# zhaihongjia/SplatLoc

Measured on AMD Instinct MI355X. Metric: fwd+bwd frames/s @1080p, 500k Gaussians, 32 feat-ch; HBM GB/s vs roofline, higher is better.
Workload: dtype f32

## Files before the change

### include/splatraster.h

```cpp
#ifndef SPLATRASTER_H
#define SPLATRASTER_H

#include <stddef.h>
#include <stdint.h>

#ifdef __cplusplus
extern "C" {
#endif

#define SPLATRASTER_ABI_VERSION 20

#define SPLATRASTER_TILE 16

#define SPLATRASTER_OK 0
#define SPLATRASTER_ERR_BAD_ARG 1
#define SPLATRASTER_ERR_HIP 2
#define SPLATRASTER_ERR_UNSUPPORTED 3
#define SPLATRASTER_ERR_OVERFLOW 4
#define SPLATRASTER_WARN_LOOKBACK_STALL 5

typedef struct splatraster_settings {
    int32_t image_height;
    int32_t image_width;
    float tanfovx;
// ... 160 lines not shown
    float* dL_drotation;
    float* dL_dopacity;
    float* dL_df_dc;
    float* dL_dextra;
    const float* reg_row_grad;
    const float* reg_out;
    float reg_weight;
} splatraster_raw_params;
int splatraster_backward_window_raw(const splatraster_settings* s, int32_t n_views, const splatraster_window_view* views,
                                    int32_t P, const int64_t* num_rendered, const float* bg, const float* means3D,
                                    const float* colors_precomp, const float* scales, const float* rotations, void* geometry,
                                    const void* binning, const void* image, const splatraster_raw_params* raw,
                                    float* dL_dmeans3D , void* stream);

typedef struct splatraster_bounded_status {
    uint32_t total;
    uint32_t overflow;
    uint32_t first_tag;
    uint32_t first_total;
    uint32_t last_tag;
    uint32_t reserved[11];
} splatraster_bounded_status;
int splatraster_bounded_status_create(void** handle);
int splatraster_bounded_status_destroy(void* handle);
int splatraster_bounded_status_read(const void* handle, splatraster_bounded_status* out);
int splatraster_bounded_status_clear(void* handle, void* stream);
int splatraster_forward_window_bounded_supported(int32_t P, int32_t n_views, int32_t width, int32_t height);
int splatraster_forward_window_bounded(const splatraster_settings* s, int32_t n_views, const splatraster_window_view* views,
                                       int32_t P, const float* means3D, const float* opacities, const float* scales,
                                       const float* rotations, const float* cov3D_precomp, const float* bg,
                                       const float* colors_precomp, void* geometry, void* binning, void* image,
                                       int64_t capacity, uint32_t tag, void* status, void* stream);
int splatraster_forward_window_bounded_raw(const splatraster_settings* s, int32_t n_views, const splatraster_window_view* views,
                                           int32_t P, const float* means3D, const splatraster_raw_forward* raw, const float* bg,
                                           void* geometry, void* binning, void* image, int64_t capacity, uint32_t tag,
                                           void* status, void* stream);


int splatraster_mark_visible(int32_t P, const float* means3D, const float* viewmatrix,
                             const float* projmatrix, uint8_t* present, void* stream);

typedef struct splatraster_geometry_layout {
    size_t rec0;
    size_t rec1;
    size_t tiles_touched;
    size_t depth_order;
    size_t offsets;
    size_t rgb;
    size_t clamped;
    size_t total;
} splatraster_geometry_layout;
typedef struct splatraster_binning_layout {
    size_t point_list;
    size_t tile_list;
    size_t ranges;
    size_t total;
} splatraster_binning_layout;
typedef struct splatraster_image_layout {
    size_t final_T;
    size_t n_contrib;
    size_t total;
} splatraster_image_layout;
int splatraster_get_geometry_layout(int32_t P, splatraster_geometry_layout* out);
int splatraster_get_binning_layout(int32_t P, int64_t R, int32_t width, int32_t height, int32_t channels,
                                   splatraster_binning_layout* out);
int splatraster_get_image_layout(int32_t width, int32_t height, splatraster_image_layout* out);
int splatraster_get_window_geometry_layout(int32_t P, int32_t n_views, splatraster_geometry_layout* out);
int splatraster_get_window_binning_layout(int32_t P, int32_t n_views, int64_t R_total, int32_t width, int32_t height,
                                          int32_t channels, splatraster_binning_layout* out);
int splatraster_get_window_image_layout(int32_t width, int32_t height, int32_t n_views, splatraster_image_layout* out);

size_t splatraster_sort_tmp_bytes(int64_t n);
int splatraster_sort_pairs_u32(int64_t n, uint32_t* keys, uint32_t* vals, int32_t key_bits,
                               void* tmp, void* stream);


int splatraster_debug_sort_path(int64_t n, int32_t key_bits, int32_t keys16);
int splatraster_debug_scan_path(int64_t n);
size_t splatraster_debug_scan_tmp_bytes(int64_t n);
int splatraster_debug_scan_u32(int64_t n, const uint32_t* in, const uint32_t* perm, uint32_t* out, uint64_t* total,
                               int32_t exclusive, uint32_t* span_owner, uint32_t span, uint32_t span_cap, void* tmp,
                               void* stream);
int splatraster_debug_sort_pairs_k16(int64_t n, uint32_t* keys, uint32_t* vals, int32_t key_bits, void* tmp, void* stream);


int splatraster_activate_forward(int32_t P, int32_t sh_coeffs, int32_t active_sh_degree,
                                 int32_t scaling_cols, int32_t extras,
                                 const float* xyz, const float* f_dc, const float* f_rest,
                                 const float* scaling, const float* rotation, const float* opacity,
                                 const float* extra, const float* campos,
                                 float* scales , float* rotations ,
                                 float* opacities , float* colors ,
                                 void* stream);
int splatraster_activate_backward(int32_t P, int32_t sh_coeffs, int32_t active_sh_degree,
                                  int32_t scaling_cols, int32_t extras,
                                  const float* xyz, const float* f_dc, const float* f_rest,
                                  const float* scaling, const float* rotation, const float* opacity,
                                  const float* campos,
                                  const float* dL_dscales, const float* dL_drotations,
                                  const float* dL_dopacities, const float* dL_dcolors,
                                  float* dL_dxyz, float* dL_df_dc, float* dL_df_rest, float* dL_dscaling,
                                  float* dL_drotation, float* dL_dopacity, float* dL_dextra, void* stream);

int splatraster_densification_stats(int32_t P, const float* viewspace_grad , const int32_t* radii,
                                    float* xyz_gradient_accum , float* denom ,
                                    float* max_radii2D , void* stream);
int splatraster_densification_stats_window(int32_t P, int32_t n_views, const float* const* viewspace_grads,
                                           const int32_t* const* radii, float* xyz_gradient_accum, float* denom,
                                           float* max_radii2D, void* stream);


typedef struct splatraster_model {
    int32_t P;
    int32_t f_rest_width;
    int32_t marker_width;
    int32_t kp_width;
    int32_t scaling_width;
    float* xyz;
    float* f_dc;
    float* f_rest;
    float* opacity;
    float* marker;
    float* kp_score;
    float* scaling;
    float* rotation;
} splatraster_model;

size_t splatraster_densify_workspace_bytes(int32_t P);
int splatraster_densify_plan(const splatraster_model* model, const float* xyz_gradient_accum ,
                             const float* denom , float max_grad, float min_opacity, float extent,
                             float percent_dense, int32_t use_size_prune, int32_t primitive_reg, void* workspace,
                             int32_t* new_P, void* stream);
int splatraster_densify_plan_thresholds(const splatraster_model* model, const float* xyz_gradient_accum ,
                                        const float* denom , float max_grad, float min_opacity,
                                        float size_split, float size_prune, int32_t use_size_prune,
                                        int32_t primitive_reg, void* workspace, int32_t* new_P, void* stream);
int splatraster_densify_apply(const splatraster_model* model, const splatraster_model* exp_avg ,
                              const splatraster_model* exp_avg_sq , const float* unit_noise ,
                              uint64_t seed, uint64_t draw_id, void* workspace , int32_t new_P,
                              splatraster_model* out_model, splatraster_model* out_exp_avg,
                              splatraster_model* out_exp_avg_sq, int32_t* source_row ,
                              int32_t* source_kind ,
                              void* stream);

int splatraster_model_append(const splatraster_model* model, const splatraster_model* exp_avg ,
                             const splatraster_model* exp_avg_sq , const splatraster_model* extra,
                             splatraster_model* out_model, splatraster_model* out_exp_avg,
                             splatraster_model* out_exp_avg_sq, void* stream);

typedef struct splatraster_adam_group {
    float* param;
    const float* grad;
    float* exp_avg;
    float* exp_avg_sq;
    const float* row_gate;
    int64_t numel;
    int32_t row_width;
    float lr;
    double step;
} splatraster_adam_group;
int splatraster_adam_step(int32_t n_groups, const splatraster_adam_group* groups, double beta1, double beta2, double eps,
                          float row_gate_threshold, void* stream);
int splatraster_adam_step_radii(int32_t n_groups, const splatraster_adam_group* groups, double beta1, double beta2, double eps,
                                float row_gate_threshold, int32_t P, const int32_t* radii, float* max_radii2D, void* stream);

int splatraster_adam_step_gated(int32_t n_groups, const splatraster_adam_group* groups, double beta1, double beta2, double eps,
// ... 285 lines not shown
```

### splatloc_amd/_native.py

```python
from __future__ import annotations

import ctypes as C
import os

from . import build as _build

_LIB = None
ABI_VERSION = 20
ERR_UNSUPPORTED = 3

OK = 0
WARN_LOOKBACK_STALL = 5
_ERR_NAMES = {1: "bad argument", 2: "HIP runtime error", 3: "unsupported configuration",
              4: "tile instance count overflow", 5: "look-back stall (results late, never wrong)"}


class Settings(C.Structure):
    _fields_ = [
        ("image_height", C.c_int32),
        ("image_width", C.c_int32),
        ("tanfovx", C.c_float),
        ("tanfovy", C.c_float),
        ("scale_modifier", C.c_float),
        ("sh_degree", C.c_int32),
# ... 74 lines not shown


class GridLayout(C.Structure):
    _fields_ = [("n_dims", C.c_int32), ("n_levels", C.c_int32), ("n_features", C.c_int32), ("grid_type", C.c_int32),
                ("offset", C.c_uint32 * GRID_MAX_LEVELS), ("size", C.c_uint32 * GRID_MAX_LEVELS),
                ("resolution", C.c_uint32 * GRID_MAX_LEVELS), ("scale", C.c_float * GRID_MAX_LEVELS), ("n_params", C.c_int64)]


DECODER_MAX_LAYERS = 8


class DecoderLayout(C.Structure):
    _fields_ = [("grid", GridLayout), ("bound", (C.c_double * 2) * 3), ("n_layers", C.c_int32),
                ("dims", C.c_int32 * (DECODER_MAX_LAYERS + 1))]


FUSION_MAX_FRAMES = 8
FUSION_MAX_FEAT_DIM = 256


class FusionVolume(C.Structure):
    _fields_ = [("dim", C.c_int32 * 3), ("feat_dim", C.c_int32), ("axis", C.c_void_p * 3), ("tsdf", C.c_void_p),
                ("weight", C.c_void_p), ("color", C.c_void_p), ("feat", C.c_void_p)]


_vp, _i32, _i64, _sz = C.c_void_p, C.c_int32, C.c_int64, C.c_size_t
SYMBOLS = {
    "splatraster_geometry_bytes": (_sz, [_i32]),
    "splatraster_binning_bytes": (_sz, [_i32, _i64, _i32, _i32, _i32]),
    "splatraster_image_bytes": (_sz, [_i32, _i32]),
    "splatraster_forward_geometry": (C.c_int, [C.POINTER(Settings), _i32] + [_vp] * 9 + [_vp, _vp, C.POINTER(_i64), _vp]),
    "splatraster_forward_render": (C.c_int, [C.POINTER(Settings), _i32, _i64] + [_vp] * 9),
    "splatraster_backward": (C.c_int, [C.POINTER(Settings), _i32, _i64] + [_vp] * 33),
    "splatraster_window_geometry_bytes": (_sz, [_i32, _i32]),
    "splatraster_window_binning_bytes": (_sz, [_i32, _i32, _i64, _i32, _i32, _i32]),
    "splatraster_window_image_bytes": (_sz, [_i32, _i32, _i32]),
    "splatraster_forward_window_geometry": (C.c_int, [C.POINTER(Settings), _i32, C.POINTER(WindowView), _i32] + [_vp] * 6
                                            + [C.POINTER(_i64), _vp]),
    "splatraster_forward_window_render": (C.c_int, [C.POINTER(Settings), _i32, C.POINTER(WindowView), _i32, C.POINTER(_i64)]
                                          + [_vp] * 6),
    "splatraster_backward_window": (C.c_int, [C.POINTER(Settings), _i32, C.POINTER(WindowView), _i32, C.POINTER(_i64)]
                                    + [_vp] * 16),
    "splatraster_window_camera_workspace_bytes": (_sz, [_i32]),
    "splatraster_backward_window_cameras": (C.c_int, [C.POINTER(Settings), _i32, C.POINTER(WindowView), _i32, C.POINTER(_i64)]
                                            + [_vp] * 14),
    "splatraster_backward_window_joint": (C.c_int, [C.POINTER(Settings), _i32, C.POINTER(WindowView), _i32, C.POINTER(_i64)]
                                          + [_vp] * 20),
    "splatraster_forward_window_geometry_raw": (C.c_int, [C.POINTER(Settings), _i32, C.POINTER(WindowView), _i32, _vp, C.POINTER(RawForward),
                                                          _vp, C.POINTER(_i64), _vp]),
    "splatraster_backward_window_raw": (C.c_int, [C.POINTER(Settings), _i32, C.POINTER(WindowView), _i32, C.POINTER(_i64)]
                                        + [_vp] * 8 + [C.POINTER(RawParams)] + [_vp] * 2),
    "splatraster_bounded_status_create": (C.c_int, [C.POINTER(_vp)]),
    "splatraster_bounded_status_destroy": (C.c_int, [_vp]),
    "splatraster_bounded_status_read": (C.c_int, [_vp, C.POINTER(BoundedStatus)]),
    "splatraster_bounded_status_clear": (C.c_int, [_vp, _vp]),
    "splatraster_forward_window_bounded_supported": (C.c_int, [_i32, _i32, _i32, _i32]),
    "splatraster_forward_window_bounded": (C.c_int, [C.POINTER(Settings), _i32, C.POINTER(WindowView), _i32] + [_vp] * 10
                                           + [_i64, C.c_uint32, _vp, _vp]),
    "splatraster_forward_window_bounded_raw": (C.c_int, [C.POINTER(Settings), _i32, C.POINTER(WindowView), _i32, _vp,
                                                         C.POINTER(RawForward)] + [_vp] * 4 + [_i64, C.c_uint32, _vp, _vp]),
    "splatraster_get_window_geometry_layout": (C.c_int, [_i32, _i32, C.POINTER(GeometryLayout)]),
    "splatraster_get_window_binning_layout": (C.c_int, [_i32, _i32, _i64, _i32, _i32, _i32, C.POINTER(BinningLayout)]),
    "splatraster_get_window_image_layout": (C.c_int, [_i32, _i32, _i32, C.POINTER(ImageLayout)]),
    "splatraster_debug_set_small_panel_max_waves": (C.c_int, [C.c_int]),
    "splatraster_debug_set_split_max_waves": (C.c_int, [C.c_int]),
    "splatraster_debug_set_fwd_team": (C.c_int, [C.c_int]),
    "splatraster_debug_set_front_end": (C.c_int, [C.c_int]),
    "splatraster_debug_set_tile_sort_cap": (C.c_int, [C.c_int]),
    "splatraster_debug_set_sort_fork": (C.c_int, [C.c_int]),
    "splatraster_debug_set_payload_stream_min": (C.c_int, [C.c_int64]),
    "splatraster_debug_set_payload_compact": (C.c_int, [C.c_int]),
    "splatraster_debug_set_dead_marks": (C.c_int, [C.c_int]),
    "splatraster_mark_visible": (C.c_int, [_i32, _vp, _vp, _vp, _vp, _vp]),
    "splatraster_get_geometry_layout": (C.c_int, [_i32, C.POINTER(GeometryLayout)]),
    "splatraster_get_binning_layout": (C.c_int, [_i32, _i64, _i32, _i32, _i32, C.POINTER(BinningLayout)]),
    "splatraster_get_image_layout": (C.c_int, [_i32, _i32, C.POINTER(ImageLayout)]),
    "splatraster_sort_tmp_bytes": (_sz, [_i64]),
    "splatraster_sort_pairs_u32": (C.c_int, [_i64, _vp, _vp, _i32, _vp, _vp]),
    "splatraster_debug_sort_path": (C.c_int, [_i64, _i32, _i32]),
    "splatraster_debug_scan_path": (C.c_int, [_i64]),
    "splatraster_debug_scan_tmp_bytes": (_sz, [_i64]),
    "splatraster_debug_scan_u32": (C.c_int, [_i64, _vp, _vp, _vp, _vp, _i32, _vp, C.c_uint32, C.c_uint32, _vp, _vp]),
    "splatraster_debug_sort_pairs_k16": (C.c_int, [_i64, _vp, _vp, _i32, _vp, _vp]),
    "splatraster_timing_enable": (C.c_int, [C.c_int]),
    "splatraster_timing_select": (C.c_int, [C.c_uint32]),
    "splatraster_timing_collect": (C.c_int, [_vp, _vp]),
    "splatknn_workspace_bytes": (_sz, [_i32]),
    "splatknn_dist2": (C.c_int, [_i32, _vp, _vp, _vp, _vp]),
    "splatknn_debug_set_grid_min": (C.c_int, [_i32]),
    "splatraster_grid_encoding_layout": (C.c_int, [_i32] * 5 + [C.c_double, _i32, C.POINTER(GridLayout)]),
    "splatraster_grid_encoding_forward": (C.c_int, [C.POINTER(GridLayout), _i64, _vp, _vp, _vp, _vp]),
    "splatraster_grid_encoding_backward": (C.c_int, [C.POINTER(GridLayout), _i64] + [_vp] * 6),
    "splatraster_decoder_workspace_bytes": (C.c_int, [C.POINTER(DecoderLayout), _i64, C.POINTER(_sz), C.POINTER(_sz)]),
    "splatraster_decoder_forward": (C.c_int, [C.POINTER(DecoderLayout), _i64, _vp, _i32, _vp, C.POINTER(_vp), _vp, _vp, _vp]),
    "splatraster_decoder_backward": (C.c_int, [C.POINTER(DecoderLayout), _i64, _vp, C.POINTER(_vp)] + [_vp] * 9),
    "splatraster_decoder_adam": (C.c_int, [C.POINTER(DecoderLayout), C.POINTER(_vp)] + [_vp] * 7 + [_i64] + [C.c_double] * 7 + [_vp]),
    "splatraster_landmark_scores": (C.c_int, [_i64, _i32] + [_vp] * 4 + [_i32, _i32] + [_vp] * 7),
    "splatraster_landmark_workspace_bytes": (_sz, [_i64, _i32]),
    "splatraster_landmark_select": (C.c_int, [_i64, _vp, _vp, _i32, C.c_double, _vp, _vp, _vp, _vp]),
    "splatraster_fusion_bytes": (C.c_int, [_i32] * 4 + [C.POINTER(_sz), C.POINTER(_sz)]),
    "splatraster_fusion_integrate": (C.c_int, [C.POINTER(FusionVolume), _i32, _i32, _i32] + [_vp] * 5 + [C.c_float, C.c_float, _vp]),
    "splatraster_fusion_surface_count": (C.c_int, [C.POINTER(FusionVolume), _i32, C.c_float, _vp, C.POINTER(_i64), _vp]),
    "splatraster_fusion_surface_extract": (C.c_int, [C.POINTER(FusionVolume), _vp, C.c_double, _vp, _i64] + [_vp] * 6),
    "splatraster_fusion_mesh_bytes": (C.c_int, [_i32] * 3 + [C.POINTER(_sz)]),
    "splatraster_fusion_mesh_count": (C.c_int, [C.POINTER(FusionVolume), _vp, _vp, C.POINTER(_i64), _vp]),
    "splatraster_fusion_mesh_extract": (C.c_int, [C.POINTER(FusionVolume), _vp, _vp, _i64, _i64, _vp, _vp, _vp]),
    "splatraster_debug_mc_table": (C.c_int, [_vp]),
    "splatraster_image_gradient": (C.c_int, [_i32] * 4 + [_vp, C.c_float, _vp, _vp, _vp, _vp]),
    "splatraster_grad_mask_workspace_bytes": (C.c_int, [_i32] * 5 + [C.POINTER(_sz)]),
    "splatraster_grad_mask": (C.c_int, [_i32] * 3 + [_vp, C.c_float, C.c_float, _i32, _i32, _vp, _vp, _vp, _vp, _sz, _vp]),
    "splatraster_debug_image_ops_path": (C.c_int, [_i32, _i32]),
    "splatraster_masked_median_workspace_bytes": (C.c_int, [_i32, _i64, C.POINTER(_sz)]),
    "splatraster_masked_median": (C.c_int, [_i32, _i64, _vp, _i32, _vp, C.c_float, _vp, _vp, _vp, _vp, _vp, _vp, _sz, _vp]),
    "splatraster_sp_nms_tile": (C.c_int, [C.POINTER(_i32), C.POINTER(_i32)]),
    "splatraster_sp_workspace_bytes": (C.c_int, [_i32] * 4 + [C.POINTER(_sz)]),
    "splatraster_sp_scores": (C.c_int, [_i32] * 3 + [_vp, _vp, _vp]),
    "splatraster_sp_nms": (C.c_int, [_i32] * 3 + [_vp, _i32, _vp, _vp]),
    "splatraster_sp_select": (C.c_int, [_i32] * 3 + [_vp, C.c_float, _i32, _i32] + [_vp] * 5 + [_sz, _vp]),
    "splatraster_sp_sample": (C.c_int, [_i32] * 3 + [_vp, _i32] + [_vp] * 4 + [_sz, _vp]),
    "splatraster_sp_dense_descriptors": (C.c_int, [_i32] * 3 + [_vp, _i32, _i32, _vp, _vp, _sz, _vp]),
    "splatraster_lsap_workspace_bytes": (_sz, [_i32, _vp]),
    "splatraster_lsap": (C.c_int, [_i32, _vp, _vp, _i32] + [_vp] * 6),
    "splatraster_debug_set_lsap_lds": (C.c_int, [C.c_int]),
    "splatraster_match_cost": (C.c_int, [_i32, _i32, _i32, _vp, _vp, C.c_float, _vp, _vp, _vp]),
    "splatraster_match_sims": (C.c_int, [_i32, _i32, _i32, _vp, _vp, _vp, C.c_float, _i64, _vp, _vp, _vp, _vp]),
    "splatraster_frustum_workspace_bytes": (_sz, [_i64, _i32, _i32]),
    "splatraster_frustum_candidates": (C.c_int, [_i64, _vp, _vp, C.c_float, _vp, _vp, _i32, _i32] + [_vp] * 10),
    "splatraster_pnp_workspace_bytes": (_sz, [_i32, _vp, _vp]),
    "splatraster_pnp": (C.c_int, [_i32] + [_vp] * 12),
    "splatraster_pnp_hypotheses": (C.c_int, [_i32, _vp, _vp, _i64, _i32] + [_vp] * 7),
    "splatraster_pnp_score": (C.c_int, [_i32, _vp, _vp, _i32] + [_vp] * 7),
    "splatraster_retrieval_workspace_bytes": (_sz, [_i64, _i64, _i32, _i32]),
    "splatraster_retrieval_topk": (C.c_int, [_i64, _i64, _i32, _i32] + [_vp] * 7),
    "splatraster_pose_errors": (C.c_int, [_i64] + [_vp] * 8),
    "splatraster_pose_invert": (C.c_int, [_i64] + [_vp] * 5),
    "splatraster_activate_forward": (C.c_int, [_i32] * 5 + [_vp] * 13),
    "splatraster_activate_backward": (C.c_int, [_i32] * 5 + [_vp] * 19),
    "splatraster_densification_stats": (C.c_int, [_i32] + [_vp] * 6),
    "splatraster_densification_stats_window": (C.c_int, [_i32, _i32] + [_vp] * 6),
    "splatraster_densify_workspace_bytes": (_sz, [_i32]),
    "splatraster_densify_plan": (C.c_int, [C.POINTER(Model), _vp, _vp, C.c_float, C.c_float, C.c_float, C.c_float, _i32,
                                           _i32, _vp, C.POINTER(_i32), _vp]),
    "splatraster_densify_plan_thresholds": (C.c_int, [C.POINTER(Model), _vp, _vp, C.c_float, C.c_float, C.c_float,
                                                      C.c_float, _i32, _i32, _vp, C.POINTER(_i32), _vp]),
    "splatraster_densify_apply": (C.c_int, [C.POINTER(Model), C.POINTER(Model), C.POINTER(Model), _vp, C.c_uint64,
                                            C.c_uint64, _vp, _i32, C.POINTER(Model), C.POINTER(Model), C.POINTER(Model),
                                            _vp, _vp, _vp]),
    "splatraster_model_append": (C.c_int, [C.POINTER(Model)] * 7 + [_vp]),
    "splatraster_adam_step": (C.c_int, [_i32, C.POINTER(AdamGroup), C.c_double, C.c_double, C.c_double, C.c_float, _vp]),
    "splatraster_adam_step_radii": (C.c_int, [_i32, C.POINTER(AdamGroup), C.c_double, C.c_double, C.c_double, C.c_float, _i32, _vp, _vp, _vp]),
    "splatraster_adam_step_gated": (C.c_int, [_i32, C.POINTER(AdamGroup), C.c_double, C.c_double, C.c_double, C.c_float, _vp, _vp]),
    "splatraster_adam_step_radii_gated": (C.c_int, [_i32, C.POINTER(AdamGroup), C.c_double, C.c_double, C.c_double, C.c_float, _i32, _vp,
                                                    _vp, _vp, _vp]),
    "splatraster_isotropic_loss_workspace_bytes": (_sz, [_i32]),
    "splatraster_isotropic_loss": (C.c_int, [_i32, _i32, _vp, _vp, _vp, _vp, _vp, _vp]),
    "splatraster_mapping_loss_workspace_bytes": (_sz, [_i32]),
    "splatraster_mapping_loss": (C.c_int, [_i32] + [_vp] * 6 + [C.c_float] + [_vp] * 7),
    "splatraster_mapping_loss_window": (C.c_int, [_i32, _i32, _vp, C.c_float, _vp, _vp, _vp]),
    "splatraster_refinement_loss_workspace_bytes": (_sz, [_i32, _i32, _i32]),
    "splatraster_refinement_loss": (C.c_int, [_i32, _i32, _i32, C.c_float] + [_vp] * 6),
    "splatraster_eval_metrics_workspace_bytes": (_sz, [_i32, _i32, _i32]),
    "splatraster_eval_metrics": (C.c_int, [_i32, _i32, _i32] + [_vp] * 5),
    "splatraster_l1_rgbd_loss": (C.c_int, [_i64, _vp, _vp, _i64, _vp, _vp, C.c_float, _vp, _vp, _vp, _vp]),
    "splatraster_pose_step": (C.c_int, [_vp] * 5 + [C.c_float] * 5 + [C.c_int] + [_vp] * 5),
    "splatraster_l1_rgbd_loss_window": (C.c_int, [_i32, C.POINTER(L1View), _i64, _i64, C.c_float, _vp, _vp]),
    "splatraster_pose_step_window": (C.c_int, [_i32] + [_vp] * 5 + [C.c_float] * 5 + [C.c_int] + [_vp] * 5),
# ... 120 lines not shown
```

### splatloc_amd/csrc/binning.hip

```cpp
#include "tile_order.h"
#include "composite_common.h"

namespace sr {

__device__ __forceinline__ int f2i_sat_b(float v)
{
    if (!(v > -1.0e9f)) v = -1.0e9f;
    if (!(v < 1.0e9f)) v = 1.0e9f;
    return (int)v;
}

constexpr int EMIT_BLOCK = 256;
constexpr int EMIT_IPT = 4;
static_assert(EMIT_SPAN == EMIT_BLOCK * EMIT_IPT, "common.h: EMIT_SPAN");

template <typename KeyT>
__global__ void __launch_bounds__(EMIT_BLOCK)
emit_kernel(int64_t R, int P , int Pv , int tiles_per_view, int W, int H,
            const uint32_t* __restrict__ offsets,
            const uint32_t* __restrict__ depth_order, const float4* __restrict__ rec,
            KeyT* __restrict__ keys, uint32_t* __restrict__ vals,
            const uint32_t* __restrict__ span_owner ,
            uint32_t* __restrict__ ranges, uint32_t nranges )
{
    for (uint32_t w = blockIdx.x * blockDim.x + threadIdx.x; w < nranges; w += gridDim.x * blockDim.x) ranges[w] = 0u;
    __shared__ uint32_t s_off[EMIT_SPAN + 1];
    __shared__ uint32_t s_gid[EMIT_SPAN], s_org[EMIT_SPAN], s_w[EMIT_SPAN];
    __shared__ int s_min;
    const int t = threadIdx.x;
    const int64_t j0 = (int64_t)blockIdx.x * EMIT_SPAN;
    const uint32_t j0u = (uint32_t)j0;
    int lo = 0, hi = P;
    if (span_owner && blockIdx.x < SPAN_OWNER_CAP) {
        lo = (int)span_owner[blockIdx.x];
        hi = lo + 1;
    }
    while (hi - lo > 1) {
        const int n = hi - lo;
        const int step = (n + EMIT_BLOCK - 1) / EMIT_BLOCK;
        if (t == 0) s_min = EMIT_BLOCK;
        __syncthreads();
        const int last = lo + (t + 1) * step - 1;
        if (last >= hi - 1 || offsets[last] > j0u) atomicMin(&s_min, t);
        __syncthreads();
        const int seg = s_min;
        __syncthreads();
        lo = lo + seg * step;
        hi = min(hi, lo + step);
    }
    const int r_lo = lo;
    for (int q = t; q <= EMIT_SPAN; q += EMIT_BLOCK) {
        const int r = r_lo - 1 + q;
        s_off[q] = r < 0 ? 0u : offsets[min(r, P - 1)];
    }
    __syncthreads();
    const int gx = (W + TILE - 1) / TILE, gy = (H + TILE - 1) / TILE;
    const uint32_t j_last = (uint32_t)(min(R, j0 + (int64_t)EMIT_SPAN) - 1);
    int nr;
    {
        int a = 1, b = EMIT_SPAN + 1;
        while (a < b) {
            const int mid = (a + b) >> 1;
            if (s_off[mid] > j_last) b = mid; else a = mid + 1;
        }
        nr = a;
    }
    for (int q = t; q < nr; q += EMIT_BLOCK) {
        const uint32_t g = depth_order[r_lo + q] & 0xFFFFFFu;
        const float4 p = rec[2 * g];
        const float rf = p.w;
        const int rminx = min(gx, max(0, f2i_sat_b((p.x - rf) / (float)TILE)));
        const int rminy = min(gy, max(0, f2i_sat_b((p.y - rf) / (float)TILE)));
        const int rmaxx = min(gx, max(0, f2i_sat_b((p.x + rf + (float)(TILE - 1)) / (float)TILE)));
        s_gid[q] = g;
        const uint32_t v = (P == Pv) ? 0u : g / (uint32_t)Pv;
        s_org[q] = v * (uint32_t)tiles_per_view + (uint32_t)rminy * (uint32_t)gx + (uint32_t)rminx;
        s_w[q] = (uint32_t)(rmaxx - rminx);
    }
    __syncthreads();
#pragma unroll
    for (int it = 0; it < EMIT_IPT; ++it) {
        const int64_t j = j0 + it * EMIT_BLOCK + t;
        if (j < R) {
            const uint32_t ju = (uint32_t)j;
            int a = 1, b = nr + 1;
            while (a < b) {
                const int mid = (a + b) >> 1;
                if (s_off[mid] > ju) b = mid; else a = mid + 1;
            }
            const uint32_t k = ju - s_off[a - 1];
            const uint32_t w = s_w[a - 1];
            const uint32_t row = k / w;
            keys[j] = (KeyT)(s_org[a - 1] + row * (uint32_t)gx + (k - row * w));
            vals[j] = s_gid[a - 1];
        }
    }
}

int launch_emit(const FramePlan& p, int64_t R, const GeomView& g, uint32_t* keys, uint32_t* vals, uint32_t* ranges,
                uint32_t nranges, hipStream_t stream, bool keys16)
{
    if (R == 0) return SPLATRASTER_OK;
    const int64_t blocks = (R + EMIT_SPAN - 1) / EMIT_SPAN;
    const int n = p.P * p.V;
    const uint32_t* owner = scan_state_bytes(n) ? g.span_owner : nullptr;
    if (keys16)
        hipLaunchKernelGGL(emit_kernel<uint16_t>, dim3((unsigned)blocks), dim3(EMIT_BLOCK), 0, stream, R, n, p.P, p.tiles, p.W, p.H,
                           g.offsets, g.depth_order, g.rec, reinterpret_cast<uint16_t*>(keys), vals, owner, ranges, nranges);
    else
        hipLaunchKernelGGL(emit_kernel<uint32_t>, dim3((unsigned)blocks), dim3(EMIT_BLOCK), 0, stream, R, n, p.P, p.tiles, p.W, p.H,
                           g.offsets, g.depth_order, g.rec, keys, vals, owner, ranges, nranges);
    SR_LAUNCH_CHECK();
    return SPLATRASTER_OK;
}

int launch_ranges_clear(int32_t tiles, uint32_t* ranges, hipStream_t stream)
{
    SR_HIP_CHECK(hipMemsetAsync(ranges, 0, sizeof(uint32_t) * 2 * (size_t)tiles, stream));
    return SPLATRASTER_OK;
}

#ifndef SR_PAYLOAD_NT_MIN
#define SR_PAYLOAD_NT_MIN (8ll << 20)
#endif
static int64_t g_payload_stream_min = SR_PAYLOAD_NT_MIN;
void set_payload_stream_min(int64_t instances) { g_payload_stream_min = instances < 0 ? (int64_t)SR_PAYLOAD_NT_MIN : instances; }

template <bool NT>
__global__ void __launch_bounds__(256)
payload_kernel(int64_t R, int gx, int tiles_per_view, int V, const uint32_t* __restrict__ point_list,
               const uint32_t* __restrict__ tile_list, const float4* __restrict__ rec,
               float4* __restrict__ irec, uint32_t* __restrict__ ipack, uint32_t* __restrict__ ranges)
{
    const int64_t j = (int64_t)blockIdx.x * blockDim.x + threadIdx.x;
    if (j >= R) return;
    const uint32_t g = point_list[j], t = tile_list[j];
    const float4 a0 = rec[2 * (size_t)g], a1 = rec[2 * (size_t)g + 1];
    uint32_t tl = t;
#pragma unroll 1
    for (int v = 1; v < V && tl >= (uint32_t)tiles_per_view; ++v) tl -= (uint32_t)tiles_per_view;
    const uint32_t ty = tl / (uint32_t)gx, tx = tl - ty * (uint32_t)gx;
    const float4 c1 = payload_conic(a1);
    const uint32_t m = g | (quadrant_reach_mask(a0, a1, (float)(tx * TILE), (float)(ty * TILE)) << 24);
    if (NT) {
        typedef float f32x4_t __attribute__((ext_vector_type(4)));
        f32x4_t* out = reinterpret_cast<f32x4_t*>(irec) + 2 * j;
        __builtin_nontemporal_store((f32x4_t){a0.x, a0.y, a0.z, a0.w}, out);
        __builtin_nontemporal_store((f32x4_t){c1.x, c1.y, c1.z, c1.w}, out + 1);
        __builtin_nontemporal_store(m, ipack + j);
    } else {
        irec[2 * j] = a0;
        irec[2 * j + 1] = c1;
        ipack[j] = m;
    }
    if (j == 0 || tile_list[j - 1] != t) ranges[2 * t] = (uint32_t)j;
    if (j == R - 1 || tile_list[j + 1] != t) ranges[2 * t + 1] = (uint32_t)(j + 1);
}

int launch_payload(const FramePlan& p, int64_t R, const GeomView& g, const BinView& b, hipStream_t stream)
{
    if (R == 0) return SPLATRASTER_OK;
    if (R >= g_payload_stream_min)
        hipLaunchKernelGGL(payload_kernel<true>, dim3((unsigned)((R + 255) / 256)), dim3(256), 0, stream, R, p.gx, p.tiles, p.V,
                           b.point_list, b.tile_list, g.rec, b.irec, b.ipack, b.ranges);
    else
        hipLaunchKernelGGL(payload_kernel<false>, dim3((unsigned)((R + 255) / 256)), dim3(256), 0, stream, R, p.gx, p.tiles, p.V,
                           b.point_list, b.tile_list, g.rec, b.irec, b.ipack, b.ranges);
    SR_LAUNCH_CHECK();
    return SPLATRASTER_OK;
}

__global__ void __launch_bounds__(256)
ranges_kernel(int64_t R, const uint32_t* __restrict__ tile_list, uint32_t* __restrict__ ranges)
{
    const int64_t j = (int64_t)blockIdx.x * blockDim.x + threadIdx.x;
    if (j >= R) return;
    const uint32_t t = tile_list[j];
    if (j == 0 || tile_list[j - 1] != t) ranges[2 * t] = (uint32_t)j;
    if (j == R - 1 || tile_list[j + 1] != t) ranges[2 * t + 1] = (uint32_t)(j + 1);
}

template <bool NT>
__global__ void __launch_bounds__(256)
payload_tile_kernel(int gx, int tiles_per_view, const uint32_t* __restrict__ ranges, const uint32_t* __restrict__ point_list,
                    const float4* __restrict__ rec, float4* __restrict__ irec, uint32_t* __restrict__ ipack,
// ... 118 lines not shown
```

### splatloc_amd/csrc/capi.hip

```cpp
#include <assert.h>
#include <string.h>

#include <mutex>
#include <unordered_map>
#include <string>
#include <vector>

#include "common.h"

namespace sr {

static thread_local std::string g_last_error;
static int g_deterministic = 0;
static int g_split_max_waves = SPLIT_MAX_WAVES;
static int g_fwd_team = -1;
static int g_payload_compact = -1;
static int g_dead_marks = 1;
static int g_bin_mode = -1;

void set_hip_error(hipError_t e, const char* what)
{
    g_last_error = std::string(what) + ": " + hipGetErrorString(e);
}

// ... 963 lines not shown
    if (P < 0) return SPLATRASTER_ERR_BAD_ARG;
    if (P == 0) return SPLATRASTER_OK;
    if (!means3D || !viewmatrix || !present) return SPLATRASTER_ERR_BAD_ARG;
    return launch_mark_visible(P, means3D, viewmatrix, present, reinterpret_cast<hipStream_t>(stream));
}

int splatraster_poll_errors(void) { return lookback_error_poll(); }

int splatraster_debug_set_deterministic(int on)
{
    g_deterministic = on ? 1 : 0;
    return SPLATRASTER_OK;
}

int splatraster_debug_set_spin_limit(uint32_t limit)
{
    int st = lookback_error_init();
    if (st) return st;
    return lookback_set_spin_limit(limit);
}

int splatraster_debug_exp2(int64_t n, const float* x, float* y, void* stream)
{
    if (n < 0) return SPLATRASTER_ERR_BAD_ARG;
    if (n == 0) return SPLATRASTER_OK;
    if (!x || !y) return SPLATRASTER_ERR_BAD_ARG;
    return launch_debug_exp2(n, x, y, reinterpret_cast<hipStream_t>(stream));
}

int splatraster_debug_poison_lds(uint32_t pattern, void* stream)
{
    return launch_poison_lds(pattern, reinterpret_cast<hipStream_t>(stream));
}

struct SortInPlace { uint32_t *keys_alt, *vals_alt; void* tmp; size_t bytes; };
static SortInPlace sort_in_place_layout(void* base, int64_t n)
{
    const size_t m = (size_t)(n > 0 ? n : 1);
    SortInPlace L;
    Carver c{base};
    L.keys_alt = c.take<uint32_t>(m);
    L.vals_alt = c.take<uint32_t>(m);
    L.tmp = c.take<char>(sort_tmp_bytes(n));
    L.bytes = c.o;
    return L;
}
size_t splatraster_sort_tmp_bytes(int64_t n) { return sort_in_place_layout(nullptr, n).bytes; }

static int sort_in_place(bool keys16, int64_t n, uint32_t* keys, uint32_t* vals, int32_t key_bits, void* tmp, void* stream_)
{
    if (!keys || !vals || !tmp) return SPLATRASTER_ERR_BAD_ARG;
    {
        int st0 = lookback_error_init();
        if (st0) return st0;
    }
    hipStream_t stream = reinterpret_cast<hipStream_t>(stream_);
    const SortInPlace L = sort_in_place_layout(tmp, n);
    uint32_t *ka = L.keys_alt, *va = L.vals_alt;
    bool in_alt = false;
    int st = keys16 ? sort_pairs_k16(n, keys, vals, ka, va, key_bits, L.tmp, stream, &in_alt)
                    : sort_pairs_u32(n, keys, vals, ka, va, key_bits, L.tmp, stream, &in_alt);
    if (st) return st;
    if (in_alt) {
        SR_HIP_CHECK(hipMemcpyAsync(keys, ka, 4 * (size_t)n, hipMemcpyDeviceToDevice, stream));
        SR_HIP_CHECK(hipMemcpyAsync(vals, va, 4 * (size_t)n, hipMemcpyDeviceToDevice, stream));
    }
    return SPLATRASTER_OK;
}

int splatraster_sort_pairs_u32(int64_t n, uint32_t* keys, uint32_t* vals, int32_t key_bits, void* tmp,
                               void* stream_)
{
    if (n < 0 || key_bits < 0 || key_bits > 32) return SPLATRASTER_ERR_BAD_ARG;
    if (n == 0 || key_bits == 0) return SPLATRASTER_OK;
    return sort_in_place(false, n, keys, vals, key_bits, tmp, stream_);
}

int splatraster_debug_sort_pairs_k16(int64_t n, uint32_t* keys, uint32_t* vals, int32_t key_bits, void* tmp, void* stream_)
{
    if (n < 0 || key_bits < 0 || key_bits > 32 || !sort_keys16(n, key_bits)) return SPLATRASTER_ERR_BAD_ARG;
    return sort_in_place(true, n, keys, vals, key_bits, tmp, stream_);
}

int splatraster_debug_sort_path(int64_t n, int32_t key_bits, int32_t keys16)
{
    if (n < 0 || key_bits < 0 || key_bits > 32 || (keys16 && !sort_keys16(n, key_bits))) return -1;
    return sort_path(n, key_bits, keys16 != 0);
}

int splatraster_debug_scan_path(int64_t n) { return n < 0 ? -1 : scan_path(n); }

size_t splatraster_debug_scan_tmp_bytes(int64_t n) { return scan_tmp_bytes(n > 0 ? n : 0); }

int splatraster_debug_scan_u32(int64_t n, const uint32_t* in, const uint32_t* perm, uint32_t* out, uint64_t* total,
                               int32_t exclusive, uint32_t* span_owner, uint32_t span, uint32_t span_cap, void* tmp, void* stream_)
{
    if (n < 0) return SPLATRASTER_ERR_BAD_ARG;
    if (exclusive && (perm || in != out || span_owner)) return SPLATRASTER_ERR_BAD_ARG;
    if (span_owner && span == 0) return SPLATRASTER_ERR_BAD_ARG;
    if (n > 0 && (!in || !out || !tmp)) return SPLATRASTER_ERR_BAD_ARG;
    if (n > 0 && perm && in == out) return SPLATRASTER_ERR_BAD_ARG;
    if (n == 0 && !total) return SPLATRASTER_OK;
    {
        int st0 = lookback_error_init();
        if (st0) return st0;
    }
    hipStream_t stream = reinterpret_cast<hipStream_t>(stream_);
    uint32_t* total32 = reinterpret_cast<uint32_t*>(total);
    if (exclusive) return exclusive_scan_u32(n, out, total32, tmp, stream, false);
    return inclusive_scan_u32(n, in, perm, out, total32, tmp, stream, false, span_owner, span, span_cap);
}

int splatraster_timing_enable(int on)
{
    std::lock_guard<std::mutex> lk(g_timing_mu);
    g_timing_mask = on ? 0xffffffffu : 0u;
    return SPLATRASTER_OK;
}

int splatraster_timing_select(uint32_t stage_mask)
{
    std::lock_guard<std::mutex> lk(g_timing_mu);
    g_timing_mask = stage_mask;
    return SPLATRASTER_OK;
}

int splatraster_timing_collect(double* ms, int64_t* counts)
{
    if (!ms || !counts) return SPLATRASTER_ERR_BAD_ARG;
    std::lock_guard<std::mutex> lk(g_timing_mu);
    for (const StageRec& r : g_recs) {
        SR_HIP_CHECK(hipEventSynchronize(r.b));
        float t = 0.f;
        SR_HIP_CHECK(hipEventElapsedTime(&t, r.a, r.b));
        if (r.stage >= 0 && r.stage < SPLATRASTER_STAGE_COUNT) { ms[r.stage] += (double)t; counts[r.stage] += 1; }
        g_pool.push_back(r.a);
        g_pool.push_back(r.b);
    }
    g_recs.clear();
    return SPLATRASTER_OK;
}

}
```

### splatloc_amd/csrc/scan.h

```cpp
#pragma once
#include "common.h"

namespace sr {

__device__ __forceinline__ uint64_t lanes_below(int lane) { return (lane == 0) ? 0ull : (~0ull >> (WAVE - lane)); }

template <typename T>
__device__ __forceinline__ T wave_inclusive_scan(T v)
{
    static_assert(sizeof(T) == 4 || sizeof(T) == 8, "uint32_t or uint64_t");
    const int lane = threadIdx.x & (WAVE - 1);
#pragma unroll
    for (int d = 1; d < WAVE; d <<= 1) {
        const T t = __shfl_up(v, d, WAVE);
        if (lane >= d) v += t;
    }
    return v;
}

template <int THREADS, typename T>
__device__ __forceinline__ T block_exclusive_scan(T v, T* s_wsum, T* total = nullptr)
{
    constexpr int NW = THREADS / WAVE;
    const int w = __builtin_amdgcn_readfirstlane(threadIdx.x / WAVE);
    const T incl = wave_inclusive_scan(v);
    if ((threadIdx.x & (WAVE - 1)) == WAVE - 1) s_wsum[w] = incl;
    __syncthreads();
    T before = 0, all = 0;
    constexpr int UNROLL = NW <= 4 ? NW : 2;
#pragma unroll UNROLL
    for (int k = 0; k < NW; ++k) {
        const T c = s_wsum[k];
        before += (k < w) ? c : (T)0;
        all += c;
    }
    if (total) *total = all;
    return before + incl - v;
}

__device__ __forceinline__ uint32_t float_order_key(float v)
{
    const uint32_t u = __float_as_uint(v);
    return (u & 0x80000000u) ? ~u : (u | 0x80000000u);
}
__device__ __forceinline__ float float_from_order_key(uint32_t key)
{
    return __uint_as_float((key & 0x80000000u) ? (key ^ 0x80000000u) : ~key);
}

template <bool DESCENDING>
__device__ __forceinline__ void radix_pick(const uint32_t* hist, bool median, uint32_t k, uint32_t* digit, uint32_t* rank, uint32_t* total)
{
    const int lane = threadIdx.x & (WAVE - 1);
    uint32_t c[4];
#pragma unroll
    for (int j = 0; j < 4; ++j) c[j] = hist[DESCENDING ? 255 - (4 * lane + j) : 4 * lane + j];
    const uint32_t s = (c[0] + c[1]) + (c[2] + c[3]);
    const uint32_t incl = wave_inclusive_scan(s);
    const uint32_t tot = __shfl(incl, WAVE - 1);
    if (median) k = tot ? (tot - 1) / 2 : 0;
    const uint32_t excl = incl - s;
    const bool mine = excl <= k && k < incl;
    uint32_t dg = 0, kr = 0;
    if (mine) {
        uint32_t cum = excl;
#pragma unroll
        for (int j = 0; j < 4; ++j) {
            if (k < cum + c[j]) {
                dg = DESCENDING ? 255 - (4 * lane + j) : 4 * lane + j;
                kr = k - cum;
                break;
            }
            cum += c[j];
        }
    }
    const unsigned long long owners = __ballot(mine);
    const int src = owners ? __ffsll((long long)owners) - 1 : 0;
    *digit = __shfl(dg, src);
    *rank = __shfl(kr, src);
    *total = tot;
}

struct plain_barrier {
    __device__ __forceinline__ void operator()() const { __syncthreads(); }
};
template <int THREADS, bool DESCENDING, typename KeyAt, typename FirstBarrier = plain_barrier>
__device__ __forceinline__ uint32_t radix_select_block(uint32_t n, KeyAt key_at, uint32_t k, uint32_t* s_hist, uint32_t* s_sel,
                                                       uint32_t* rank_left = nullptr, FirstBarrier first_barrier = FirstBarrier())
{
    static_assert(THREADS >= 256, "one thread per bin");
    const uint32_t tid = threadIdx.x;
    uint32_t prefix = 0;
    for (int shift = 24; shift >= 0; shift -= 8) {
        if (tid < 256) s_hist[tid] = 0;
        __syncthreads();
        const uint32_t hi = shift == 24 ? 0u : 0xFFFFFFFFu << (shift + 8);
        for (uint32_t i = tid; i < n; i += THREADS) {
            const uint32_t u = key_at(i);
// ... 24 lines not shown
```

Measured before the change: 798.3.

## Replace per-instance binary search in emit with owner-mark max-scan and reciprocal division

The tile-key emit kernel no longer binary-searches the shared offset array for each output slot. Each range start now writes its owner index into a 16-bit shared array, and a wave-level inclusive max-scan plus a cross-wave carry spreads ownership to every slot. The per-instance integer division that splits an index into row and column is replaced by a float reciprocal estimate with a one-step correction when the tile count is small enough. A debug C entry point is added to test emit on its own. The aim is to cut the log-depth shared-memory searches and the slow integer divides. The costs are extra shared-memory passes and barriers, and a new limit on grid width that returns unsupported.

```diff
diff --git a/include/splatraster.h b/include/splatraster.h
--- a/include/splatraster.h
+++ b/include/splatraster.h
@@ -266,6 +266,8 @@
                                int32_t exclusive, uint32_t* span_owner, uint32_t span, uint32_t span_cap, void* tmp,
                                void* stream);
 int splatraster_debug_sort_pairs_k16(int64_t n, uint32_t* keys, uint32_t* vals, int32_t key_bits, void* tmp, void* stream);
+int splatraster_debug_emit(int64_t R, int32_t n, int32_t Pv, int32_t W, int32_t H, const uint32_t* offsets, const uint32_t* depth_order,
+                           const float* rec, uint32_t* keys, uint32_t* vals, int32_t keys16, const uint32_t* span_owner, void* stream);
 
 
 int splatraster_activate_forward(int32_t P, int32_t sh_coeffs, int32_t active_sh_degree,
diff --git a/splatloc_amd/_native.py b/splatloc_amd/_native.py
--- a/splatloc_amd/_native.py
+++ b/splatloc_amd/_native.py
@@ -180,6 +180,7 @@
     "splatraster_debug_scan_tmp_bytes": (_sz, [_i64]),
     "splatraster_debug_scan_u32": (C.c_int, [_i64, _vp, _vp, _vp, _vp, _i32, _vp, C.c_uint32, C.c_uint32, _vp, _vp]),
     "splatraster_debug_sort_pairs_k16": (C.c_int, [_i64, _vp, _vp, _i32, _vp, _vp]),
+    "splatraster_debug_emit": (C.c_int, [_i64, _i32, _i32, _i32, _i32, _vp, _vp, _vp, _vp, _vp, _i32, _vp, _vp]),
     "splatraster_timing_enable": (C.c_int, [C.c_int]),
     "splatraster_timing_select": (C.c_int, [C.c_uint32]),
     "splatraster_timing_collect": (C.c_int, [_vp, _vp]),
diff --git a/splatloc_amd/csrc/binning.hip b/splatloc_amd/csrc/binning.hip
--- a/splatloc_amd/csrc/binning.hip
+++ b/splatloc_amd/csrc/binning.hip
@@ -13,6 +13,18 @@
 constexpr int EMIT_BLOCK = 256;
 constexpr int EMIT_IPT = 4;
 static_assert(EMIT_SPAN == EMIT_BLOCK * EMIT_IPT, "common.h: EMIT_SPAN");
+static_assert(EMIT_SPAN <= 65536 && EMIT_BLOCK == 4 * WAVE, "emit_kernel: 16-bit row numbers, one 64-slot segment per wave and step");
+
+constexpr uint32_t EMIT_RCP_MAX_TILES = 1u << 22;
+__device__ __forceinline__ uint32_t rect_row(uint32_t k, uint32_t w, uint32_t* col)
+{
+    uint32_t row = (uint32_t)(((float)k + 0.5f) * __builtin_amdgcn_rcpf((float)w));
+    int32_t c = (int32_t)(k - row * w);
+    if (c < 0) { row -= 1u; c += (int32_t)w; }
+    else if (c >= (int32_t)w) { row += 1u; c -= (int32_t)w; }
+    *col = (uint32_t)c;
+    return row;
+}
 
 template <typename KeyT>
 __global__ void __launch_bounds__(EMIT_BLOCK)
@@ -25,7 +37,9 @@
 {
     for (uint32_t w = blockIdx.x * blockDim.x + threadIdx.x; w < nranges; w += gridDim.x * blockDim.x) ranges[w] = 0u;
     __shared__ uint32_t s_off[EMIT_SPAN + 1];
-    __shared__ uint32_t s_gid[EMIT_SPAN], s_org[EMIT_SPAN], s_w[EMIT_SPAN];
+    __shared__ uint32_t s_gid[EMIT_SPAN], s_org[EMIT_SPAN];
+    __shared__ uint16_t s_w[EMIT_SPAN];
+    __shared__ uint16_t s_own[EMIT_SPAN];
     __shared__ int s_min;
     const int t = threadIdx.x;
     const int64_t j0 = (int64_t)blockIdx.x * EMIT_SPAN;
@@ -53,19 +67,15 @@
         const int r = r_lo - 1 + q;
         s_off[q] = r < 0 ? 0u : offsets[min(r, P - 1)];
     }
+#pragma unroll
+    for (int it = 0; it < EMIT_IPT; ++it) s_own[it * EMIT_BLOCK + t] = 0;
     __syncthreads();
     const int gx = (W + TILE - 1) / TILE, gy = (H + TILE - 1) / TILE;
     const uint32_t j_last = (uint32_t)(min(R, j0 + (int64_t)EMIT_SPAN) - 1);
-    int nr;
-    {
-        int a = 1, b = EMIT_SPAN + 1;
-        while (a < b) {
-            const int mid = (a + b) >> 1;
-            if (s_off[mid] > j_last) b = mid; else a = mid + 1;
-        }
-        nr = a;
-    }
-    for (int q = t; q < nr; q += EMIT_BLOCK) {
+    for (int q = t; q < EMIT_SPAN; q += EMIT_BLOCK) {
+        const uint32_t start = s_off[q];
+        if (start > j_last || s_off[q + 1] == start) continue;
+        s_own[start > j0u ? start - j0u : 0u] = (uint16_t)q;
         const uint32_t g = depth_order[r_lo + q] & 0xFFFFFFu;
         const float4 p = rec[2 * g];
         const float rf = p.w;
@@ -75,25 +85,41 @@
         s_gid[q] = g;
         const uint32_t v = (P == Pv) ? 0u : g / (uint32_t)Pv;
         s_org[q] = v * (uint32_t)tiles_per_view + (uint32_t)rminy * (uint32_t)gx + (uint32_t)rminx;
-        s_w[q] = (uint32_t)(rmaxx - rminx);
+        s_w[q] = (uint16_t)(rmaxx - rminx);
     }
     __syncthreads();
+    const int wave = __builtin_amdgcn_readfirstlane(t / WAVE);
+#pragma unroll
+    for (int it = 0; it < EMIT_IPT; ++it) {
+        const int sl = it * EMIT_BLOCK + t;
+        s_own[sl] = (uint16_t)wave_inclusive_max_scan((uint32_t)s_own[sl]);
+    }
+    __syncthreads();
+    uint32_t carry = 0;
+    for (int k = 0; k < wave; ++k) carry = max(carry, (uint32_t)__builtin_amdgcn_readfirstlane((int)s_own[k * WAVE + WAVE - 1]));
+    const bool by_rcp = (uint32_t)tiles_per_view <= EMIT_RCP_MAX_TILES;
 #pragma unroll
     for (int it = 0; it < EMIT_IPT; ++it) {
         const int64_t j = j0 + it * EMIT_BLOCK + t;
         if (j < R) {
             const uint32_t ju = (uint32_t)j;
-            int a = 1, b = nr + 1;
-            while (a < b) {
-                const int mid = (a + b) >> 1;
-                if (s_off[mid] > ju) b = mid; else a = mid + 1;
+            const uint32_t a = max((uint32_t)s_own[it * EMIT_BLOCK + t], carry);
+            const uint32_t k = ju - s_off[a];
+            const uint32_t w = s_w[a];
+            uint32_t row, col;
+            if (by_rcp) {
+                row = rect_row(k, w, &col);
+            } else {
+                row = k / w;
+                col = k - row * w;
             }
-            const uint32_t k = ju - s_off[a - 1];
-            const uint32_t w = s_w[a - 1];
-            const uint32_t row = k / w;
-            keys[j] = (KeyT)(s_org[a - 1] + row * (uint32_t)gx + (k - row * w));
-            vals[j] = s_gid[a - 1];
+            keys[j] = (KeyT)(s_org[a] + row * (uint32_t)gx + col);
+            vals[j] = s_gid[a];
         }
+        if (it + 1 < EMIT_IPT)
+#pragma unroll
+            for (int d = 0; d < EMIT_BLOCK / WAVE; ++d)
+                carry = max(carry, (uint32_t)__builtin_amdgcn_readfirstlane((int)s_own[((it * (EMIT_BLOCK / WAVE) + wave + d) * WAVE) + WAVE - 1]));
     }
 }
 
@@ -101,6 +127,7 @@
                 uint32_t nranges, hipStream_t stream, bool keys16)
 {
     if (R == 0) return SPLATRASTER_OK;
+    if (p.gx > 65535) return SPLATRASTER_ERR_UNSUPPORTED;
     const int64_t blocks = (R + EMIT_SPAN - 1) / EMIT_SPAN;
     const int n = p.P * p.V;
     const uint32_t* owner = scan_state_bytes(n) ? g.span_owner : nullptr;
diff --git a/splatloc_amd/csrc/capi.hip b/splatloc_amd/csrc/capi.hip
--- a/splatloc_amd/csrc/capi.hip
+++ b/splatloc_amd/csrc/capi.hip
@@ -1069,6 +1069,30 @@
     return sort_in_place(true, n, keys, vals, key_bits, tmp, stream_);
 }
 
+int splatraster_debug_emit(int64_t R, int32_t n, int32_t Pv, int32_t W, int32_t H, const uint32_t* offsets, const uint32_t* depth_order,
+                           const float* rec, uint32_t* keys, uint32_t* vals, int32_t keys16, const uint32_t* span_owner, void* stream_)
+{
+    if (R < 0 || R >= ((int64_t)1 << 31) || n < 1 || Pv < 1 || n % Pv || n / Pv > MAX_VIEWS || W < 1 || H < 1 || !offsets || !depth_order ||
+        !rec || !keys || !vals)
+        return SPLATRASTER_ERR_BAD_ARG;
+    FramePlan p{};
+    p.W = W;
+    p.H = H;
+    p.gx = (W + TILE - 1) / TILE;
+    p.gy = (H + TILE - 1) / TILE;
+    p.tiles = p.gx * p.gy;
+    p.P = Pv;
+    p.V = n / Pv;
+    p.gtiles = (int64_t)p.V * p.tiles;
+    if (keys16 && p.gtiles > 65536) return SPLATRASTER_ERR_BAD_ARG;
+    GeomView g{};
+    g.offsets = const_cast<uint32_t*>(offsets);
+    g.depth_order = const_cast<uint32_t*>(depth_order);
+    g.rec = reinterpret_cast<float4*>(const_cast<float*>(rec));
+    g.span_owner = const_cast<uint32_t*>(span_owner);
+    return launch_emit(p, R, g, keys, vals, nullptr, 0u, reinterpret_cast<hipStream_t>(stream_), keys16 != 0);
+}
+
 int splatraster_debug_sort_path(int64_t n, int32_t key_bits, int32_t keys16)
 {
     if (n < 0 || key_bits < 0 || key_bits > 32 || (keys16 && !sort_keys16(n, key_bits))) return -1;
diff --git a/splatloc_amd/csrc/scan.h b/splatloc_amd/csrc/scan.h
--- a/splatloc_amd/csrc/scan.h
+++ b/splatloc_amd/csrc/scan.h
@@ -14,6 +14,17 @@
     for (int d = 1; d < WAVE; d <<= 1) {
         const T t = __shfl_up(v, d, WAVE);
         if (lane >= d) v += t;
+    }
+    return v;
+}
+
+__device__ __forceinline__ uint32_t wave_inclusive_max_scan(uint32_t v)
+{
+    const int lane = threadIdx.x & (WAVE - 1);
+#pragma unroll
+    for (int d = 1; d < WAVE; d <<= 1) {
+        const uint32_t t = __shfl_up(v, d, WAVE);
+        if (lane >= d) v = max(v, t);
     }
     return v;
 }
```

Result: no change. 796.7 (-0.2%).
